# mobilinkd/m17-cxx-demod

Hardware: AMD Instinct MI355X
Metric: Msamples/s demodulated (48 kSPS 4-FSK in -> decoded frames) (higher is better)
Workload: dtype f32

## Files before the change

m17-cxx-demod_amd/csrc/m17_decode_device.hpp:

```cpp
#pragma once

#include "m17_common.hpp"

namespace m17 {

struct DecodeTables {
    uint16_t src[8][488];
    uint16_t lich_src[96];
    uint32_t golay_fix[2048];
};

__device__ __constant__ const int DEC_IN[4] = {488, 296, 420, 402};
__device__ __constant__ const int DEC_OUT[4] = {240, 144, 206, 197};

struct DecodeLds {
    uint32_t* llr;
    uint32_t* hist;
    uint32_t* outb;
    uint32_t* lsf;
    const uint16_t* src;
    const uint16_t* lich_src;
    int stride;
    int32_t* soft;
    unsigned long long* prof;
};

#define M17_LDS __attribute__((address_space(3)))
typedef uint32_t v4u __attribute__((ext_vector_type(4)));
template <typename T> __device__ __forceinline__ M17_LDS T* as_lds(T* p) { return (M17_LDS T*)p; }
template <typename T> __device__ __forceinline__ const M17_LDS T* as_lds(const T* p) { return (const M17_LDS T*)p; }
#define M17_GLOBAL __attribute__((address_space(1)))
template <typename T> __device__ __forceinline__ M17_GLOBAL T* as_global(T* p) { return (M17_GLOBAL T*)p; }
template <typename T> __device__ __forceinline__ T lds_get(const M17_LDS T* p)
{
    static_assert(sizeof(T) % 4 == 0, "word-sized structs only");
    T v;
    const M17_LDS uint32_t* s = reinterpret_cast<const M17_LDS uint32_t*>(p);
    uint32_t* d = reinterpret_cast<uint32_t*>(&v);
#pragma unroll
    for (int k = 0; k < (int)(sizeof(T) / 4); ++k) d[k] = s[k];
    return v;
}
template <typename T> __device__ __forceinline__ void lds_put(M17_LDS T* p, const T& v)
{
    static_assert(sizeof(T) % 4 == 0, "word-sized structs only");
    M17_LDS uint32_t* d = reinterpret_cast<M17_LDS uint32_t*>(p);
    const uint32_t* s = reinterpret_cast<const uint32_t*>(&v);
#pragma unroll
    for (int k = 0; k < (int)(sizeof(T) / 4); ++k) d[k] = s[k];
}

__device__ __forceinline__ int llr_at(const uint32_t* llr, int stride, int lane, int idx)
{
    const uint32_t w = llr[(idx >> 2) * stride + lane];
    return (int)(int8_t)(w >> (8 * (idx & 3)));
}
template <bool LQ = false>
__device__ __forceinline__ int llr_at_nib(const uint32_t* llr, int stride, int lane, int idx)
{
    const uint32_t w = LQ ? as_lds(llr)[(idx >> 3) * stride + lane] : llr[(idx >> 3) * stride + lane];
    return (int)(((w >> (4 * (idx & 7))) & 0xFu) ^ 8u) - 8;
}
template <bool NIB = false, bool LQ = false>
__device__ __forceinline__ int soft_at(const uint16_t* src, const uint32_t* llr, int stride, int lane, int kind, int i, int stale)
{
    const uint32_t e = LQ ? as_lds(src)[kind * 488 + i] : src[kind * 488 + i];
    if (LQ) {
        const int v = NIB ? llr_at_nib<LQ>(llr, stride, lane, (int)(e & 0x1FFu)) : llr_at(llr, stride, lane, (int)(e & 0x1FFu));
        const int w = (e & 0x200u) ? -v : v;
        return (e & 0x8000u) ? 0 : ((e & 0x4000u) ? stale : w);
    }
    if (e & 0x8000u) return 0;
    if (e & 0x4000u) return stale;
    const int v = NIB ? llr_at_nib<LQ>(llr, stride, lane, (int)(e & 0x1FFu)) : llr_at(llr, stride, lane, (int)(e & 0x1FFu));
    return (e & 0x200u) ? -v : v;
}
__device__ __forceinline__ uint32_t pack_llr_nibbles(uint32_t lo, uint32_t hi)
{
    auto four = [](uint32_t w) { return (w & 0xFu) | ((w >> 4) & 0xF0u) | ((w >> 8) & 0xF00u) | ((w >> 12) & 0xF000u); };
    return four(lo) | (four(hi) << 16);
}
__device__ __forceinline__ uint32_t unpack_llr_nibbles(uint32_t packed, int half)
{
    const uint32_t h = half ? packed >> 16 : packed & 0xFFFFu;
    uint32_t w = 0;
    for (int q = 0; q < 4; ++q) {
        const uint32_t n = (h >> (4 * q)) & 0xFu;
        w |= ((uint32_t)(uint8_t)(int8_t)((int)(n ^ 8u) - 8)) << (8 * q);
    }
    return w;
}
__device__ __forceinline__ uint32_t byte_at(const uint32_t* col, int stride, int lane, int b)
{
    return (col[(b >> 2) * stride + lane] >> (8 * (b & 3))) & 0xFFu;
}

__device__ __forceinline__ uint32_t crc16_col(const uint32_t* col, int stride, int lane, int n)
{
    uint32_t reg = 0xFFFFu;
    for (int i = 0; i != 16; ++i) {
        const uint32_t bit = reg & 1u;
        if (bit) reg ^= 0x5935u;
        reg >>= 1;
        if (bit) reg |= 0x8000u;
    }
    for (int k = 0; k < n; ++k) {
        const uint32_t byte = byte_at(col, stride, lane, k);
        for (int i = 0; i != 8; ++i) {
            const uint32_t msb = reg & 0x8000u;
            reg = ((reg << 1) & 0xFFFFu) | ((byte >> (7 - i)) & 1u);
            if (msb) reg ^= 0x5935u;
        }
    }
    for (int i = 0; i != 16; ++i) {
        const uint32_t msb = reg & 0x8000u;
        reg = (reg << 1) & 0xFFFFu;
        if (msb) reg ^= 0x5935u;
    }
    return reg;
}

__device__ __forceinline__ uint32_t golay_syndrome(uint32_t cw)
{
    cw &= 0xFFFFFFu;
    for (int i = 0; i != 12; ++i) {
        if (cw & 1u) cw ^= 0xC75u;
        cw >>= 1;
    }
    return cw;
}
__device__ __forceinline__ bool golay_decode(const DecodeTables* tb, uint32_t input, uint32_t& output)
{
    const uint32_t syn = golay_syndrome(input >> 1);
    const uint32_t correction = tb->golay_fix[syn & 0x7FFu] << 1;
    output = input ^ correction;
    return __popc(syn) < 3 || !(__popc(output) & 1);
}

template <bool NIB = false, bool LQ = false>
__device__ __forceinline__ uint32_t viterbi_decode(const DecodeTables* tb, const DecodeLds& L, int lane, int kind, int& stale_io)
{
    const int IN = DEC_IN[kind & 3], OUT = DEC_OUT[kind & 3];
    const int steps = IN >> 1;
    constexpr int32_t MAXM = 0x7FFFFFFF / 2;
    int32_t m[16];
#pragma unroll
    for (int s = 0; s < 16; ++s) m[s] = MAXM;
    m[0] = 0;
    uint32_t prev_bits = 0;
    int ns0 = soft_at<NIB, LQ>(L.src, L.llr, L.stride, lane, kind, 0, stale_io);
    int ns1 = soft_at<NIB, LQ>(L.src, L.llr, L.stride, lane, kind, 1, stale_io);
    for (int h = 0; h < steps; ++h) {
        const int s0 = ns0, s1 = ns1;
        if (2 * h == 400 && (kind & 3) != 3) stale_io = s1;
        if (h + 1 < steps) {
            ns0 = soft_at<NIB, LQ>(L.src, L.llr, L.stride, lane, kind, 2 * h + 2, stale_io);
            ns1 = soft_at<NIB, LQ>(L.src, L.llr, L.stride, lane, kind, 2 * h + 3, stale_io);
        }
        const int a = s0 ? abs(-7 - s0) : 0, b = s0 ? abs(7 - s0) : 0;
        const int d = s1 ? abs(-7 - s1) : 0, e = s1 ? abs(7 - s1) : 0;
        const uint32_t nn = 2u * (uint32_t)(a + d), np = 2u * (uint32_t)(a + e), pn = 2u * (uint32_t)(b + d), pp = 2u * (uint32_t)(b + e);
        const uint32_t c0[8] = {nn, np, np, nn, pn, pp, pp, pn};
        const uint32_t c1[8] = {pp, pn, pn, pp, np, nn, nn, np};
        uint32_t n[16];
        uint32_t bits = 0;
#pragma unroll
        for (int j = 0; j < 8; ++j) {
            const uint32_t lo = (uint32_t)m[j] << 1, hi = ((uint32_t)m[j + 8] << 1) + 1u;
            const uint32_t n0 = min(lo + c0[j], hi + c1[j]);
            const uint32_t n1 = min(lo + c1[j], hi + c0[j]);
            bits = __builtin_amdgcn_alignbit(n0, bits, 1);
            bits = __builtin_amdgcn_alignbit(n1, bits, 1);
            n[2 * j] = n0 >> 1;
            n[2 * j + 1] = n1 >> 1;
        }
#pragma unroll
        for (int s = 0; s < 16; ++s) m[s] = (int32_t)n[s];
        if (h & 1) {
            const uint32_t hw = prev_bits | (bits & 0xFFFF0000u);
            if (LQ) as_global(L.hist)[(h >> 1) * L.stride + lane] = hw;
            else L.hist[(h >> 1) * L.stride + lane] = hw;
        } else prev_bits = bits >> 16;
    }
    if (steps & 1) {
        if (LQ) as_global(L.hist)[(steps >> 1) * L.stride + lane] = prev_bits;
        else L.hist[(steps >> 1) * L.stride + lane] = prev_bits;
    }
    int best = 0;
    int32_t best_cost = m[0];
#pragma unroll
    for (int s = 1; s < 16; ++s)
        if (m[s] < best_cost) { best_cost = m[s]; best = s; }
    const uint32_t cost = (uint32_t)roundf((float)best_cost / 7.0f);
#pragma unroll
    for (int q = 0; q < 8; ++q) {
        if (LQ) as_lds(L.outb)[q * L.stride + lane] = 0;
        else L.outb[q * L.stride + lane] = 0;
    }
    uint32_t state = (uint32_t)best;
    uint32_t word = 0;
    int o = OUT;
    int index = steps;
    for (int hi = steps; hi > 0 && o > 0;) {
        --hi;
        const uint32_t hw = LQ ? as_global(L.hist)[(hi >> 1) * L.stride + lane] : L.hist[(hi >> 1) * L.stride + lane];
        const uint32_t hb = (hi & 1) ? (hw >> 16) : (hw & 0xFFFFu);
        const uint32_t v = (hb >> state) & 1u;
        if (index-- <= OUT) {
            --o;
            const int byte = o >> 3;
            word |= (state & 1u) << (8 * (byte & 3) + (7 - (o & 7)));
            if ((o & 31) == 0) {
                if (LQ) as_lds(L.outb)[(byte >> 2) * L.stride + lane] = word;
                else L.outb[(byte >> 2) * L.stride + lane] = word;
                word = 0;
            }
        }
        state = (state >> 1) + (v ? 8u : 0u);
    }
    return cost;
}

__device__ __forceinline__ uint32_t pk_add_bcast_lo(uint32_t p, uint32_t c)
{
    uint32_t r;
    asm("v_pk_add_u16 %0, %1, %2 op_sel:[0,0] op_sel_hi:[0,1]" : "=v"(r) : "v"(p), "v"(c));
    return r;
}
__device__ __forceinline__ uint32_t pk_add_bcast_hi(uint32_t p, uint32_t c)
{
    uint32_t r;
    asm("v_pk_add_u16 %0, %1, %2 op_sel:[1,0] op_sel_hi:[1,1]" : "=v"(r) : "v"(p), "v"(c));
    return r;
}
__device__ __forceinline__ uint32_t pk_min_u16(uint32_t a, uint32_t b)
{
    uint32_t r;
    asm("v_pk_min_u16 %0, %1, %2" : "=v"(r) : "v"(a), "v"(b));
    return r;
}
__device__ __forceinline__ uint32_t sad_u32(uint32_t a, uint32_t b, uint32_t c)
{
    uint32_t r;
    asm("v_sad_u32 %0, %1, %2, %3" : "=v"(r) : "v"(a), "v"(b), "v"(c));
    return r;
}
__device__ __forceinline__ uint32_t pk_sub_u16(uint32_t a, uint32_t b)
{
    uint32_t r;
    asm("v_pk_sub_u16 %0, %1, %2" : "=v"(r) : "v"(a), "v"(b));
    return r;
}
__device__ __forceinline__ uint32_t viterbi_decode_pk(const DecodeLds& L, int lane, int kind, int& stale_io)
{
    const int IN = DEC_IN[kind & 3], OUT = DEC_OUT[kind & 3];
    const int steps = IN >> 1;
    constexpr uint32_t SENT = 20000u;
    uint32_t P[8];
#pragma unroll
    for (int k = 0; k < 8; ++k) P[k] = SENT | (SENT << 16);
    P[0] = SENT << 16;
    const M17_LDS uint32_t* map2 = as_lds(reinterpret_cast<const uint32_t*>(L.src)) + kind * 244;
    const M17_LDS uint32_t* frame = as_lds(L.llr);
    auto ld_e = [&](int h) -> uint32_t { return h < steps ? map2[h] : 0x80008000u; };
    auto ld_w = [&](uint32_t e16) -> uint32_t { return frame[((e16 & 0x1FFu) >> 3) * L.stride + lane]; };
    auto mk_s = [&](uint32_t e16, uint32_t w) -> int {
        const int v = (int)(((w >> (4u * (e16 & 7u))) & 0xFu) ^ 8u) - 8;
        const int wv = (e16 & 0x200u) ? -v : v;
        return (e16 & 0x8000u) ? 0 : ((e16 & 0x4000u) ? stale_io : wv);
    };
    uint32_t e_cur = ld_e(0), e_nxt = ld_e(1);
    uint32_t wa = ld_w(e_cur & 0xFFFFu), wb = ld_w(e_cur >> 16);
    for (int h = 0; h < steps; ++h) {
        const int s0 = mk_s(e_cur & 0xFFFFu, wa), s1 = mk_s(e_cur >> 16, wb);
        if (2 * h == 400 && (kind & 3) != 3) stale_io = s1;
        const uint32_t e_nn2 = ld_e(h + 2);
        wa = ld_w(e_nxt & 0xFFFFu); wb = ld_w(e_nxt >> 16);
        e_cur = e_nxt; e_nxt = e_nn2;
        const uint32_t u0 = (uint32_t)(s0 + 8), u1 = (uint32_t)(s1 + 8);
        const uint32_t r0n = s0 ? 1u : u0, r0p = s0 ? 15u : u0, r1n = s1 ? 1u : u1, r1p = s1 ? 15u : u1;
        const uint32_t a = sad_u32(u0, r0n, 0u), b = sad_u32(u0, r0p, 0u);
        const uint32_t nn = sad_u32(u1, r1n, a), np = sad_u32(u1, r1p, a), pn = sad_u32(u1, r1n, b), pp = sad_u32(u1, r1p, b);
        const uint32_t e_nn = nn | (pp << 16), e_np = np | (pn << 16), e_pn = pn | (np << 16), e_pp = pp | (nn << 16);
        const uint32_t ce[8] = {e_nn, e_np, e_np, e_nn, e_pn, e_pp, e_pp, e_pn};
        const uint32_t co[8] = {e_pp, e_pn, e_pn, e_pp, e_np, e_nn, e_nn, e_np};
        uint32_t N[8];
        uint32_t acc = 0;
#pragma unroll
        for (int j = 0; j < 8; ++j) {
            const uint32_t x = (j & 1) ? pk_add_bcast_hi(P[j >> 1], ce[j]) : pk_add_bcast_lo(P[j >> 1], ce[j]);
            const uint32_t y = (j & 1) ? pk_add_bcast_hi(P[(j + 8) >> 1], co[j]) : pk_add_bcast_lo(P[(j + 8) >> 1], co[j]);
            N[j] = pk_min_u16(x, y);
            acc = (acc >> 1) | (pk_sub_u16(y, x) & 0x80008000u);
        }
#pragma unroll
        for (int k = 0; k < 8; ++k) P[k] = N[k];
        as_global(L.hist)[h * L.stride + lane] = acc;
    }
    auto metric = [&](int s) { return (int32_t)((s & 1) ? P[s >> 1] >> 16 : P[s >> 1] & 0xFFFFu); };
    int best = 0;
    int32_t best_cost = metric(0);
#pragma unroll
    for (int s = 1; s < 16; ++s) { const int32_t v = metric(s); if (v < best_cost) { best_cost = v; best = s; } }
    const uint32_t cost = (uint32_t)roundf((float)best_cost / 7.0f);
#pragma unroll
    for (int q = 0; q < 8; ++q) as_lds(L.outb)[q * L.stride + lane] = 0;
    uint32_t state = (uint32_t)best, word = 0;
    int o = OUT, index = steps;
    for (int top = steps; top > 0 && o > 0; top -= 16) {
        uint32_t hwv[16];
#pragma unroll
        for (int i = 0; i < 16; ++i) hwv[i] = as_global(L.hist)[max(top - 1 - i, 0) * L.stride + lane];
#pragma unroll
        for (int i = 0; i < 16; ++i) {
            if (top - 1 - i < 0 || o <= 0) break;
            const uint32_t v = (hwv[i] >> (8u + (state >> 1) + ((state & 1u) << 4))) & 1u;
            if (index-- <= OUT) {
                --o;
                const int byte = o >> 3;
                word |= (state & 1u) << (8 * (byte & 3) + (7 - (o & 7)));
                if ((o & 31) == 0) { as_lds(L.outb)[(byte >> 2) * L.stride + lane] = word; word = 0; }
            }
            state = (state >> 1) + (v ? 8u : 0u);
        }
    }
    return cost;
}

__device__ __forceinline__ void wave_lds_sync()
{
    __builtin_amdgcn_fence(__ATOMIC_RELEASE, "wavefront", "local");
    __builtin_amdgcn_wave_barrier();
    __builtin_amdgcn_fence(__ATOMIC_ACQUIRE, "wavefront", "local");
}
__device__ __forceinline__ int vit_pos_of_lane(int wl) { return (wl & 15) ^ ((wl & 4) ? 3 : 0); }
__device__ __forceinline__ int vit_lane_of_pos(int p) { return p ^ ((p & 4) ? 3 : 0); }
__device__ __forceinline__ int rotl4(int v, int r) { r &= 3; return ((v << r) | (v >> (4 - r))) & 15; }
__device__ __forceinline__ int rotr4(int v, int r) { return rotl4(v, 4 - (r & 3)); }

template <int R>
__device__ __forceinline__ int32_t vit_partner(int32_t m)
{
    if constexpr (R == 3) return __builtin_amdgcn_update_dpp(0, m, 0xB1, 0xF, 0xF, true);
    else if constexpr (R == 2) return __builtin_amdgcn_update_dpp(0, m, 0x4E, 0xF, 0xF, true);
    else if constexpr (R == 1) return __builtin_amdgcn_update_dpp(0, m, 0x141, 0xF, 0xF, true);
    else return __builtin_amdgcn_update_dpp(0, m, 0x128, 0xF, 0xF, true);
}

template <int R>
__device__ __forceinline__ uint32_t vit_step(uint32_t W, int wl, int32_t& m, uint32_t sh, unsigned long long upper)
{
    const int32_t c_own = (int32_t)__builtin_amdgcn_ubfe(W, sh, 8u);
    const int32_t c_oth = (int32_t)__builtin_amdgcn_ubfe(W, 24u - sh, 8u);
    const int32_t mp = vit_partner<R>(m);
    const int32_t own = m + c_own, oth = mp + c_oth;
    const int32_t low = ((upper >> wl) & 1ull) ? oth : own;
    m = min(own, oth);
    return (uint32_t)__ballot(m != low);
}

__device__ __forceinline__ uint32_t viterbi_decode_wave(const DecodeLds& L, int wl, int kind, int& stale_io)
{
    const int IN = DEC_IN[kind & 3], OUT = DEC_OUT[kind & 3];
    const int steps = IN >> 1;
    constexpr int32_t MAXM = 0x7FFFFFFF / 2;
    const unsigned long long tp0 = L.prof ? wall_clock64() : 0ull;
    M17_LDS uint32_t* cw = as_lds(reinterpret_cast<uint32_t*>(L.soft));
    M17_LDS uint32_t* hist = as_lds(L.hist);
    M17_LDS uint32_t* outb = as_lds(L.outb);
    {
        const uint16_t* src = L.src + kind * 488;
        const M17_LDS uint32_t* llr = as_lds(L.llr);
        auto soft = [&](uint32_t e) -> int {
            if (e & 0x8000u) return 0;
            if (e & 0x4000u) return stale_io;
            const uint32_t idx = e & 0x1FFu;
            const int v = (int)(int8_t)(llr[idx >> 2] >> (8 * (idx & 3)));
            return (e & 0x200u) ? -v : v;
        };
        int wlo = wl;
        asm volatile("" : "+v"(wlo));
        uint32_t e0 = wlo < steps ? src[2 * wlo] : 0x8000u, e1 = wlo < steps ? src[2 * wlo + 1] : 0x8000u;
        for (int h = wlo; h < steps; h += 64) {
            const int hn = h + 64;
            const uint32_t n0 = hn < steps ? src[2 * hn] : 0x8000u, n1 = hn < steps ? src[2 * hn + 1] : 0x8000u;
            const int s0 = soft(e0), s1 = soft(e1);
            const int a = s0 ? abs(-7 - s0) : 0, b = s0 ? abs(7 - s0) : 0;
            const int d = s1 ? abs(-7 - s1) : 0, e = s1 ? abs(7 - s1) : 0;
            cw[h] = (uint32_t)(a + d) | ((uint32_t)(a + e) << 8) | ((uint32_t)(b + d) << 16) | ((uint32_t)(b + e) << 24);
            if (h == 200) cw[480] = (uint32_t)s1;
            e0 = n0; e1 = n1;
        }
    }
    for (int h = steps + wl; h < ((steps + 3) & ~3); h += 64) cw[h] = 0;
    wave_lds_sync();
    if ((kind & 3) != 3 && IN > 401) stale_io = (int)cw[480];
    const int pos = vit_pos_of_lane(wl);
    uint32_t sh[4];
    unsigned long long upper[4];
#pragma unroll
    for (int r = 0; r < 4; ++r) {
        const int pb = 3 - r;
        upper[r] = __ballot((pos >> pb) & 1);
        const int j = rotl4(pos & ~(1 << pb), r);
        const bool c0neg = j < 4, c1neg = (((j ^ (j >> 1)) & 1) == 0);
        sh[r] = 8u * ((c0neg ? 0u : 2u) | (c1neg ? 0u : 1u));
    }
    int32_t m = (pos == 0) ? 0 : MAXM;
    const unsigned long long tp1 = L.prof ? wall_clock64() : 0ull;
    const int groups = (steps + 3) >> 2;
    v4u Wn = *reinterpret_cast<const M17_LDS v4u*>(cw);
    if (wl < 16)
    for (int g = 0; g < groups; ++g) {
        const v4u W = Wn;
        if (g + 1 < groups) Wn = *reinterpret_cast<const M17_LDS v4u*>(cw + 4 * (g + 1));
        const int h = 4 * g;
        const uint32_t b0 = vit_step<0>(W.x, wl, m, sh[0], upper[0]);
        int32_t m1 = m, m2, m3;
        const uint32_t b1 = vit_step<1>(W.y, wl, m1, sh[1], upper[1]);
        m2 = m1;
        const uint32_t b2 = vit_step<2>(W.z, wl, m2, sh[2], upper[2]);
        m3 = m2;
        const uint32_t b3 = vit_step<3>(W.w, wl, m3, sh[3], upper[3]);
        const int left = steps - h;
        m = left >= 4 ? m3 : (left == 3 ? m2 : (left == 2 ? m1 : m));
        hist[2 * g] = b0 | (b1 << 16);
        hist[2 * g + 1] = b2 | (b3 << 16);
    }
    const unsigned long long tp2 = L.prof ? wall_clock64() : 0ull;
    int best = 0;
    int32_t best_cost = __builtin_amdgcn_readlane(m, __builtin_amdgcn_readfirstlane(vit_lane_of_pos(rotr4(0, steps))));
#pragma unroll
    for (int s = 1; s < 16; ++s) {
        const int32_t v = __builtin_amdgcn_readlane(m, __builtin_amdgcn_readfirstlane(vit_lane_of_pos(rotr4(s, steps))));
        if (v < best_cost) { best_cost = v; best = s; }
    }
    const uint32_t cost = (uint32_t)roundf((float)best_cost / 7.0f);
    wave_lds_sync();
    for (int q = wl; q < 8; q += 64) outb[q] = 0;
    {
        auto to_pos_order = [](uint32_t x) -> uint32_t {
            const uint32_t odd = x & 0xF0F0F0F0u;
            return (x & 0x0F0F0F0Fu) | ((odd & 0x10101010u) << 3) | ((odd & 0x20202020u) << 1) | ((odd >> 1) & 0x20202020u) | ((odd >> 3) & 0x10101010u);
        };
        const int nreal = (steps + 1) >> 1;
        for (int q = wl; q < 130; q += 64) {
            const uint32_t neutral = (q & 1) ? 0xAAAACCCCu : 0xF0F0FF00u;
            uint32_t x = neutral;
            if (q < nreal) {
                x = to_pos_order(hist[q]);
                if (2 * q + 1 >= steps) x = (x & 0xFFFFu) | (neutral & 0xFFFF0000u);
            }
            cw[q] = x;
        }
    }
    wave_lds_sync();
    uint32_t I = (uint32_t)wl & 15u, w4 = 0, w4_hi = 0;
    {
        const M17_LDS uint32_t* hp = cw + 32 * (wl >> 4) + 2;
        auto rotr = [](uint32_t x, uint32_t n) -> uint32_t { return __builtin_amdgcn_alignbit(x, x, n); };
        auto take = [&](uint32_t prerot, uint32_t bit) {
            const uint32_t r = rotr(prerot, I);
            uint32_t out;
            asm("v_bfi_b32 %0, %1, %2, %3" : "=v"(out) : "v"(bit), "v"(r), "v"(I));
            I = out;
        };
#pragma unroll
        for (int g = 0; g < 16; ++g) {
            const uint32_t wa = hp[31 - 2 * g], wb = hp[30 - 2 * g];
// ... 234 lines not shown
```

m17-cxx-demod_amd/csrc/m17_parity_kernels.hpp:

```cpp
#pragma once

#include "m17_common.hpp"
#include "m17_decode_device.hpp"
#include "m17_state.hpp"

namespace m17 {

__global__ __launch_bounds__(64) void slice_kernel(const float* __restrict__ sym, uint32_t rows, uint32_t n, int8_t* __restrict__ llr,
                                                   float* __restrict__ evm, const float* __restrict__ edges)
{
    const uint32_t r = blockIdx.x * 64 + threadIdx.x;
    if (r >= rows) return;
    float S = 0.f;
    const float alpha = (float)(1.0 / 184);
    for (uint32_t k = 0; k < n; ++k) {
        const float sample = sym[(size_t)r * n + k];
        const uint32_t pair = slice_llr(sample, edges);
        llr[((size_t)r * n + k) * 2] = (int8_t)(pair & 0xFF);
        llr[((size_t)r * n + k) * 2 + 1] = (int8_t)(pair >> 8);
        float e;
        if (sample > 2.f) e = sample - 3.f;
        else if (sample > 0.f) e = sample - 1.f;
        else if (sample > -2.f) e = sample + 1.f;
        else e = sample + 3.f;
        S = S - S * alpha;
        S = S + (e * e) * alpha;
        evm[(size_t)r * n + k] = sqrtf(S);
    }
}

__global__ __launch_bounds__(64) void kalman_kernel(const float* __restrict__ z, const uint32_t* __restrict__ dt, uint32_t rows, uint32_t n, int wrap,
                                                    float z0, uint32_t order, float* __restrict__ out, const core::Kalman2Gain* __restrict__ gain)
{
    __shared__ Kal2 st[64];
    const uint32_t r = blockIdx.x * 64 + threadIdx.x;
    if (r >= rows) return;
    if (wrap == -1) {
        float x0 = z0, x1 = 0.f;
        for (uint32_t i = 0; i < n; ++i) {
            core::level_update(x0, x1, z[(size_t)r * n + i], gain[min(i, (uint32_t)core::LEVEL_SCHED_LAST)], order);
            float* o = out + ((size_t)r * n + i) * 6;
            o[0] = x0; o[1] = x1; o[2] = 0.f; o[3] = 0.f; o[4] = 0.f; o[5] = 0.f;
        }
        return;
    }
    M17_LDS Kal2* kp = as_lds(&st[threadIdx.x]);
    Kal2 k;
    kal_reset(k, z0);
    lds_put(kp, k);
    for (uint32_t i = 0; i < n; ++i) {
        kal_update(kp, z[(size_t)r * n + i], dt[(size_t)r * n + i], wrap, order);
        k = lds_get(kp);
        float* o = out + ((size_t)r * n + i) * 6;
        o[0] = k.x0; o[1] = k.x1; o[2] = k.p00; o[3] = k.p01; o[4] = k.p10; o[5] = k.p11;
    }
}

__global__ __launch_bounds__(64) void viterbi_kernel(const int8_t* __restrict__ soft, uint32_t n_frames, int kind,
                                                     uint8_t* __restrict__ bits, int32_t* __restrict__ cost,
                                                     const DecodeTables* ident)
{
    extern __shared__ __attribute__((aligned(16))) uint32_t lds[];
    DecodeLds L;
    L.llr = lds;
    L.hist = lds + 122 * 64;
    L.outb = L.hist + 122 * 64;
    L.lsf = L.outb + 8 * 64;
    L.stride = 64;
    L.prof = nullptr;
    L.src = &ident->src[0][0];
    L.lich_src = ident->lich_src;
    const int lane = threadIdx.x;
    const uint32_t f = blockIdx.x * 64 + lane;
    const int IN = DEC_IN[kind], OUT = DEC_OUT[kind];
    if (f < n_frames) {
        const int8_t* src = soft + (size_t)f * IN;
        for (int k = 0; k < (IN + 3) / 4; ++k) {
            uint32_t w = 0;
            for (int q = 0; q < 4; ++q)
                if (4 * k + q < IN) w |= (uint32_t)(uint8_t)src[4 * k + q] << (8 * q);
            L.llr[k * 64 + lane] = w;
        }
        int stale = llr_at(L.llr, 64, lane, kind == 3 ? 401 : 0);
        const uint32_t cst = viterbi_decode(ident, L, lane, kind + 4, stale);
        cost[f] = (int32_t)cst;
        for (int n = 0; n < OUT; ++n) bits[(size_t)f * OUT + n] = (uint8_t)((byte_at(L.outb, 64, lane, n >> 3) >> (7 - (n & 7))) & 1u);
    }
}

struct DecodeFramesParams {
    const int8_t* llr;
    const uint8_t* sync_type;
    uint8_t* state_io;
    uint8_t* lich_io;
    uint8_t* lsf_io;
    int8_t* dep401_io;
    int64_t* cost_io;
    FrameRec* recs;
    uint8_t* nrec;
    uint32_t n;
    const DecodeTables* tables;
    uint32_t* overflow;
};

__global__ __launch_bounds__(64) void decode_frames_kernel(DecodeFramesParams P)
{
    extern __shared__ __attribute__((aligned(16))) uint32_t lds[];
    DecodeLds L;
    L.llr = lds;
    L.hist = lds + 92 * 64;
    L.outb = L.hist + 122 * 64;
    L.lsf = L.outb + 8 * 64;
    L.stride = 64;
    L.prof = nullptr;
    L.src = &P.tables->src[0][0];
    L.lich_src = P.tables->lich_src;
    const int lane = threadIdx.x;
    const uint32_t f = blockIdx.x * 64 + lane;
    if (f >= P.n) return;
    const int8_t* src = P.llr + (size_t)f * 368;
    for (int k = 0; k < 92; ++k) {
        uint32_t w = 0;
        for (int q = 0; q < 4; ++q) w |= (uint32_t)(uint8_t)src[4 * k + q] << (8 * q);
        L.llr[k * 64 + lane] = w;
    }
    for (int k = 0; k < 8; ++k) {
        uint32_t w = 0;
        for (int q = 0; q < 4; ++q)
            if (4 * k + q < 30) w |= (uint32_t)P.lsf_io[(size_t)f * 30 + 4 * k + q] << (8 * q);
        L.lsf[k * 64 + lane] = w;
    }
    DecoderRegs D{P.state_io[f], P.lich_io[f], (int)P.dep401_io[f]};
    const int64_t cin = P.cost_io[f];
    uint32_t cost = cin < 0 ? 0xFFFFFFFFu : (uint32_t)cin;
    uint32_t n_run = 0, seq = 0;
    RecSink S{P.recs + (size_t)f * 2, 2, nullptr, nullptr, f, 0, P.sync_type[f], P.overflow};
    cost = decode_frame(P.tables, L, lane, P.sync_type[f], D, cost, S, n_run, seq);
    P.state_io[f] = (uint8_t)D.state;
    P.lich_io[f] = (uint8_t)D.lich_segments;
    P.dep401_io[f] = (int8_t)D.stale401;
    P.cost_io[f] = cost == 0xFFFFFFFFu ? (int64_t)-1 : (int64_t)cost;
    P.nrec[f] = (uint8_t)n_run;
    for (int k = 0; k < 30; ++k) P.lsf_io[(size_t)f * 30 + k] = (uint8_t)byte_at(L.lsf, 64, lane, k);
}

struct DeferParams {
    FrameRec* recs;
    uint32_t rec_cap;
    const uint32_t* rec_count;
    const uint32_t* defer;
    uint32_t* hist;
    const DecodeTables* tables;
    SeqState* state;
    Diag* diag_log;
    uint32_t diag_cap;
    const uint32_t* diag_count;
    uint32_t C;
    EvParams ev;
};
constexpr int DEFER_HIST_WORDS = 201;
constexpr int DEFER_CPB = 2;
constexpr int DEFER_WAVE_WORDS = (46 + 8) * 64 + 512 / 2;
constexpr int DEFER_LDS_BYTES = DEFER_CPB * DEFER_WAVE_WORDS * 4 + 4 * 488 * 2;
constexpr uint32_t defer_blocks(uint32_t C) { return (C + DEFER_CPB - 1) / DEFER_CPB; }
__global__ __launch_bounds__(64 * DEFER_CPB) void decode_deferred_kernel(DeferParams P)
{
    extern __shared__ __attribute__((aligned(16))) uint32_t lds[];
    if (blockIdx.x >= defer_blocks(P.C)) {
        if (threadIdx.x < 64) evm_fold_pass(P.ev, blockIdx.x - defer_blocks(P.C), reinterpret_cast<float*>(lds));
        return;
    }
    const int wave = __builtin_amdgcn_readfirstlane((int)(threadIdx.x >> 6));
    uint32_t* wb = lds + wave * DEFER_WAVE_WORDS;
    DecodeLds L;
    L.llr = wb;
    L.outb = wb + 46 * 64;
    uint16_t* list = reinterpret_cast<uint16_t*>(L.outb + 8 * 64);
    uint16_t* maps = reinterpret_cast<uint16_t*>(lds + DEFER_CPB * DEFER_WAVE_WORDS);
    L.lsf = nullptr;
    L.stride = 64;
    L.prof = nullptr;
    L.soft = nullptr;
    const int lane = threadIdx.x & 63;
    const uint32_t c = blockIdx.x * DEFER_CPB + wave;
    L.hist = P.hist + (size_t)c * DEFER_HIST_WORDS * 64;
    for (int k = threadIdx.x; k < 4 * 488; k += 64 * DEFER_CPB) maps[k] = P.tables->src[k / 488][k % 488];
    __syncthreads();
    L.src = maps;
    L.lich_src = P.tables->lich_src;
    if (c >= P.C) return;
    FrameRec* recs = P.recs + (size_t)c * P.rec_cap;
    const uint32_t n = min(P.rec_count[c], P.rec_cap);
    for (uint32_t s0 = 0; s0 < n; s0 += 512) {
        const uint32_t s1 = min(n, s0 + 512u);
        uint32_t nd = 0;
        wave_lds_sync();
        for (uint32_t base = s0; base < s1; base += 64) {
            const uint32_t slot = base + lane;
            bool d = false;
            if (slot < s1) {
                const uint32_t* w = reinterpret_cast<const uint32_t*>(recs + slot);
                d = cost_is_deferred(w[4]) && w[15] == DEFER_MARK;
            }
            const unsigned long long mask = __ballot(d);
            if (d) list[nd + __popcll(mask & ((1ull << lane) - 1ull))] = (uint16_t)(slot - s0);
            nd += (uint32_t)__popcll(mask);
        }
        wave_lds_sync();
        for (uint32_t k0 = lane; k0 < nd; k0 += 64) {
            const uint32_t slot = s0 + as_lds(list)[k0];
            uint32_t* w = reinterpret_cast<uint32_t*>(recs + slot);
            const uint32_t* src = P.defer + ((size_t)c * P.rec_cap + slot) * 46;
            for (int k = 0; k < 46; ++k) as_lds(L.llr)[k * 64 + lane] = src[k];
            const int kind = kind_of_frame_type(w[5] & 0xFFu);
            int stale = (int)w[14];
            const uint32_t cost = viterbi_decode_pk(L, lane, kind, stale);
            complete_record(w, cost, L.outb, 64, lane, len_of_kind(kind));
        }
    }
    __threadfence_block();
    wave_lds_sync();
    auto settle = [&](int32_t& v) {
        const uint32_t u = (uint32_t)v;
        if (cost_is_deferred(u)) v = recs[u & ~DEFER_TAG].cost;
    };
    if (P.diag_log) {
        const uint32_t nd = min(P.diag_count[c], P.diag_cap);
        Diag* log = P.diag_log + (size_t)c * P.diag_cap;
        for (uint32_t e = lane; e < nd; e += 64) settle(log[e].viterbi_cost);
    }
}

struct SettleParams {
    FrameRec* recs; uint32_t rec_cap; const uint32_t* defer; const DecodeTables* tables; SeqState* state; uint32_t C;
    EvParams ev;
};
constexpr int SETTLE_LDS_BYTES = (92 + 122 + 8 + 488) * 4 > EV_TILE_FLOATS * 4 ? (92 + 122 + 8 + 488) * 4 : EV_TILE_FLOATS * 4;
__global__ __launch_bounds__(64) void settle_tail_kernel(SettleParams P)
{
    extern __shared__ __attribute__((aligned(16))) uint32_t lds[];
    if (blockIdx.x >= P.C) {
        evm_fold_pass(P.ev, blockIdx.x - P.C, reinterpret_cast<float*>(lds));
        return;
    }
    const int wl = threadIdx.x;
    const uint32_t c = blockIdx.x;
    SeqState* st = P.state + c;
    const uint32_t th = (uint32_t)__builtin_amdgcn_readfirstlane((int)st->hot.viterbi_cost);
    const uint32_t td = (uint32_t)__builtin_amdgcn_readfirstlane(st->cold.diag.viterbi_cost);
    if (!cost_is_deferred(th) && !cost_is_deferred(td)) return;
    DecodeLds L;
    L.llr = lds; L.hist = lds + 92; L.outb = lds + 92 + 122; L.soft = reinterpret_cast<int32_t*>(lds + 92 + 122 + 8);
    L.lsf = nullptr; L.prof = nullptr; L.stride = 1;
    L.src = &P.tables->src[0][0]; L.lich_src = P.tables->lich_src;
    auto resolve = [&](uint32_t tag) -> uint32_t {
        const uint32_t slot = tag & ~DEFER_TAG;
        if (slot >= P.rec_cap) return 0u;
        uint32_t* w = reinterpret_cast<uint32_t*>(P.recs + (size_t)c * P.rec_cap + slot);
        const uint32_t have = (uint32_t)__builtin_amdgcn_readfirstlane((int)w[4]);
        if (!cost_is_deferred(have)) return have;
        const int kind = kind_of_frame_type(w[5] & 0xFFu);
        int stale = (int)w[14];
        const uint32_t* src = P.defer + ((size_t)c * P.rec_cap + slot) * 46;
        for (int k = wl; k < 92; k += 64) as_lds(L.llr)[k] = unpack_llr_nibbles(src[k >> 1], k & 1);
        wave_lds_sync();
        const uint32_t cost = viterbi_decode_wave(L, wl, kind, stale);
        wave_lds_sync();
        if (wl == 0) complete_record(w, cost, L.outb, 1, 0, len_of_kind(kind));
        wave_lds_sync();
        return cost;
    };
    uint32_t ch = th, cd = td;
    if (cost_is_deferred(th)) ch = resolve(th);
    if (cost_is_deferred(td)) cd = (td == th) ? ch : resolve(td);
    if (wl == 0) {
        st->hot.viterbi_cost = ch;
        st->cold.diag.viterbi_cost = (int32_t)cd;
    }
}

}
```

m17-cxx-demod_amd/csrc/m17hip.hip:

```cpp
#include "../../include/m17hip.h"

#include "m17_common.hpp"
#include "m17_decode_device.hpp"
#include "m17_frontend_kernels.hpp"
#include "m17_state.hpp"
#include "m17_wave_kernel.hpp"
#include "m17_gate_kernel.hpp"
#include "m17_mod_kernels.hpp"
#include "m17_parity_kernels.hpp"
#include "m17_gather.hpp"

#include <hip/hip_ext.h>

#include <algorithm>
#include <cmath>
#include <complex>
#include <cstdio>
#include <cstdlib>
#include <cstring>
#include <ctime>
#include <mutex>
#include <new>
#include <vector>

// ... 180 lines not shown
    uint32_t diag_cap = 0;
    uint32_t kalman_order = 3;
    int gather_fault = 0;
    uint32_t gather_timeout_ms = 120000;
    uint32_t channel_base = 0;
    uint32_t front_first = 0;
    int redo_form = 0;
    int dcd_form = -1;
    uint64_t seen_overlap = 0;
    hipEvent_t last_end = nullptr;
    uint32_t seg_len = 48000;
    uint32_t seg0_len = 0;
    int64_t seg_ramp = -1;
    DevBuf<DcdState> dcd_state;
    DevBuf<SeqState> seq_state;
    struct RecSet {
        DevBuf<FrameRec> recs;
        DevBuf<uint32_t> rec_count;
        DevBuf<uint32_t> defer_llr;
        uint32_t* ovf = nullptr;
        Event chain;
        Event done;
        uint32_t C = 0, rec_cap = 0, nseg = 0;
        bool valid = false;
        bool pending = false;
        bool bert = false, pkt = false;
    } sets[2];
    int cur = 0;
    uint32_t sel_back = 0;
    bool streams() const { return copy && slab[1].x; }
    hipStream_t pay() const { return streams() ? copy : stream; }
    Event ev_dst;
    Event ev_switch;
    Event ev_fetch;
    DevBuf<uint32_t> overflow;
    DevBuf<uint64_t> rec_offsets;
    DevBuf<FrameRec> compact;
    DevBuf<DecodeTables> tables;
    DevBuf<float> taps;
    DevBuf<float> taps_skew;
    int limit_form = 1;
    int fir_form = 1;
    int gate_aware = -1;
    DevBuf<GateTruth> truth;
    DevBuf<uint32_t> first_needed;
    uint32_t off_segs_prev = 0, chan_segs_prev = 0;
    uint32_t fir_grid = 0;
    uint32_t n_cu = 256;
    DevBuf<uint32_t> defer_hist;
    bool defer_decode = true;
    bool defer_evm = true;
    DevBuf<float> ev_ops2[2];
    int ev_par = 0;
    const float* fold_ops = nullptr;
    uint32_t fold_C = 0;
    const uint32_t* fold_end = nullptr;
    uint32_t ev_pitch = 0;
    uint32_t ev_pitch_override = 0;
    DevBuf<uint32_t> ev_cur;
    bool fold_pending = false;
    DevBuf<EvState> ev_state;
    uint32_t seq_lds_bytes = 0;
    DevBuf<float> llr_edges;
    DevBuf<core::Kalman2Gain> level_gain;
    DevBuf<char> scratch;
    DcdCoef coef{};
    uint64_t pos = 0;
    std::vector<uint32_t> marks;
    std::vector<uint8_t> marked;
    TurnTable reset_list;
    std::vector<uint8_t> pol_host;
    uint32_t pol_ones = 0;
    bool pol_dirty = false;
    TurnTable pol_table;
    uint32_t lastC = 0;
    bool have_run = false;
    bool uploaded = false;
    bool timing = false;
    bool profile = false;
    DevBuf<unsigned long long> dbg;
    uint32_t dbg_waves = 0;
    std::vector<TimedLaunch> pending;
    std::vector<Event> pool;
    double acc_ms[KT_N] = {0};
    uint64_t acc_n[KT_N] = {0};
};

struct m17hip_comm {
    ncclComm_t comm = nullptr;
    int device = 0;
    int rank = 0, nranks = 1;
    int last_rccl = 0;
    DevBuf<uint64_t> counts_dev;
    uint64_t* words_host = nullptr;
    uint32_t serial = 0;
    DevBuf<char> gathered;
    bool dead = false;
};

namespace {

#define HIPCHK(ctx, expr)                                   \
    do {                                                    \
        hipError_t e_ = (expr);                             \
        if (e_ != hipSuccess) {                             \
            (ctx)->last_hip = (int)e_;                      \
            return M17HIP_EHIP;                             \
        }                                                   \
    } while (0)

size_t round_up(size_t v, size_t m) { return (v + m - 1) / m * m; }

int alloc_code(m17hip_ctx* c, hipError_t e)
{
    if (e == hipSuccess) return M17HIP_OK;
    c->last_hip = (int)e;
    return e == hipErrorOutOfMemory ? M17HIP_ENOMEM : M17HIP_EHIP;
}

const uint8_t DC_SEQ[46] = {0xd6, 0xb5, 0xe2, 0x30, 0x82, 0xFF, 0x84, 0x62, 0xba, 0x4e, 0x96, 0x90, 0xd8, 0x98, 0xdd, 0x5d,
                            0x0c, 0xc8, 0x52, 0x43, 0x91, 0x1d, 0xf8, 0x6e, 0x68, 0x2F, 0x35, 0xda, 0x14, 0xea, 0xcd, 0x76,
                            0x19, 0x8d, 0xd5, 0x80, 0xd1, 0x33, 0x87, 0x13, 0x57, 0x18, 0x2d, 0x29, 0x78, 0xc3};

uint16_t frame_source(size_t deinterleaved_index)
{
    const size_t i = deinterleaved_index;
    const size_t src = (45 * i + 92 * i * i) % 368;
    const bool neg = (DC_SEQ[src >> 3] >> (7 - (src & 7))) & 1;
    return (uint16_t)(src | (neg ? 0x200u : 0u));
}

void build_tables(DecodeTables& t)
{
    std::memset(&t, 0, sizeof(t));
    std::vector<int> p1(61), p2(12, 1), p3(8, 1);
    for (size_t i = 0, j = 2; i != 61; ++i) { if (i == j) { p1[i] = 0; j += 4; } else p1[i] = 1; }
    p2[11] = 0;
    p3[7] = 0;
    struct Lay { int out, in, first; const std::vector<int>* p; };
    const Lay lay[4] = {{488, 368, 0, &p1}, {296, 272, 96, &p2}, {420, 368, 0, &p3}, {402, 368, 0, &p2}};
    for (int k = 0; k < 4; ++k) {
        size_t index = 0, pindex = 0;
        for (int i = 0; i < 488; ++i) t.src[k][i] = 0x8000;
        int i = 0;
        for (; i != lay[k].out && index < (size_t)lay[k].in; ++i) {
            if (!(*lay[k].p)[pindex++]) t.src[k][i] = 0x8000;
            else t.src[k][i] = frame_source(lay[k].first + index++);
            if (pindex == lay[k].p->size()) pindex = 0;
        }
        for (; i < lay[k].out; ++i) t.src[k][i] = 0x4000;
        for (int q = 0; q < 488; ++q) t.src[4 + k][q] = (uint16_t)q;
    }
    for (int i = 0; i < 96; ++i) t.lich_src[i] = frame_source(i);
    auto syndrome = [](uint32_t cw) { cw &= 0xFFFFFFu; for (int i = 0; i != 12; ++i) { if (cw & 1u) cw ^= 0xC75u; cw >>= 1; } return cw; };
    std::vector<int> seen(2048, 0);
    auto put = [&](uint32_t v) { const uint32_t s = syndrome(v) & 0x7FF; t.golay_fix[s] = v; seen[s]++; };
    put(0);
    for (int i = 0; i < 23; ++i) put(1u << i);
    for (int i = 0; i < 22; ++i) for (int j = i + 1; j < 23; ++j) put((1u << i) | (1u << j));
    for (int i = 0; i < 21; ++i) for (int j = i + 1; j < 22; ++j) for (int k = j + 1; k < 23; ++k) put((1u << i) | (1u << j) | (1u << k));
}

void build_llr_edges(float* e)
{
    const float inc = (float)(1.0 / (double)7.0f);
    float k = (float)(-3.0 + (double)inc);
    for (int n = 0; n < 43; ++n) { e[n] = k; k = k + inc; }
}

DcdCoef build_coef()
{
    const std::complex<float> j{0, 1};
    const float pi2 = (float)(M_PI * 2.0);
    auto coeff = [&](size_t f) { const float k = float(f) / float(48000); return std::exp(-j * pi2 * k); };
    const auto c0 = coeff(2400), c1 = coeff(3600);
    return DcdCoef{c0.real(), c0.imag(), c1.real(), c1.imag()};
}

Event get_event(m17hip_ctx* c)
{
    Event e;
    if (!c->pool.empty()) { e = std::move(c->pool.back()); c->pool.pop_back(); return e; }
    const hipError_t r = e.create(hipEventDefault);
    if (r != hipSuccess) c->last_hip = (int)r;
    return e;
}
void pool_events(m17hip_ctx* c, Event& a, Event& b)
{
    if (a) c->pool.push_back(std::move(a));
    if (b) c->pool.push_back(std::move(b));
}
struct Timed {
    m17hip_ctx* c; int which; hipStream_t st; Event a, b;
    Timed(m17hip_ctx* ctx, int w, hipStream_t stream) : c(ctx), which(w), st(stream)
    {
        if (!c->timing) return;
        a = get_event(c); b = get_event(c);
        if (!a || !b || hipEventRecord(a, st) != hipSuccess) pool_events(c, a, b);
    }
    Timed(m17hip_ctx* ctx, int w) : Timed(ctx, w, ctx->stream) {}
    ~Timed()
    {
        if (!a) return;
        if (hipEventRecord(b, st) == hipSuccess) c->pending.push_back({std::move(a), std::move(b), which});
        else pool_events(c, a, b);
    }
};
struct TimedK {
    m17hip_ctx* c; int which; Event a, b;
    TimedK(m17hip_ctx* ctx, int w) : c(ctx), which(w)
    {
        if (!c->timing) return;
        a = get_event(c); b = get_event(c);
        if (!a || !b) pool_events(c, a, b);
    }
    ~TimedK() { if (a) c->pending.push_back({std::move(a), std::move(b), which}); }
    template <typename... P, typename... A>
    void launch(void (*kernel)(P...), dim3 grid, dim3 block, uint32_t lds, hipStream_t st, const A&... args)
    {
        if (a) hipExtLaunchKernelGGL(kernel, grid, block, lds, st, a, b, 0, static_cast<P>(args)...);
        else hipLaunchKernelGGL(kernel, grid, block, lds, st, static_cast<P>(args)...);
    }
};
struct DeviceGuard {
    int prev = -1; bool ok = true;
    explicit DeviceGuard(m17hip_ctx* c)
    {
        if (hipGetDevice(&prev) != hipSuccess) prev = -1;
        if (prev != c->device) { const hipError_t e = hipSetDevice(c->device); if (e != hipSuccess) { c->last_hip = (int)e; ok = false; prev = -1; } }
        else prev = -1;
        (void)hipGetLastError();
    }
    ~DeviceGuard() { if (prev >= 0) hipSetDevice(prev); }
};
#define GUARD(ctx) DeviceGuard guard_(ctx); if (!guard_.ok) return M17HIP_EHIP

struct RunRegistry { std::mutex mu; std::vector<m17hip_ctx*> ctxs; uint64_t overlaps = 0; };
RunRegistry& g_runs_ref() { static RunRegistry* r = new RunRegistry; return *r; }
#define g_runs (g_runs_ref())
bool runs_overlap(m17hip_ctx* c)
{
    std::lock_guard<std::mutex> lk(g_runs.mu);
    bool other = false;
    for (m17hip_ctx* o : g_runs.ctxs)
        if (o != c && o->device == c->device && o->last_end && hipEventQuery(o->last_end) == hipErrorNotReady) other = true;
    (void)hipGetLastError();
    if (other) ++g_runs.overlaps;
    const bool overlapped = other || g_runs.overlaps != c->seen_overlap;
    c->seen_overlap = g_runs.overlaps;
    return overlapped;
}
void drain_timing(m17hip_ctx* c)
{
    for (auto& t : c->pending) {
        hipEventSynchronize(t.b);
        float ms = 0.f;
        if (hipEventElapsedTime(&ms, t.a, t.b) == hipSuccess) { c->acc_ms[t.which] += ms; c->acc_n[t.which]++; }
        pool_events(c, t.a, t.b);
    }
    c->pending.clear();
}

__global__ void ev_move_kernel(SeqState* st, EvState* es, uint32_t C, int to_deferred)
{
    const uint32_t c = blockIdx.x * blockDim.x + threadIdx.x;
    if (c >= C) return;
    if (to_deferred) { es[c].S = st[c].hot.evm_S; es[c].pos = 0; } else st[c].hot.evm_S = es[c].S;
}

__device__ __forceinline__ void fresh_demod_state(SeqState* st, EvState* es, uint32_t c, uint64_t pos)
{
    es[c] = EvState{1.0f, 0.f, 0u, 0u};
    uint32_t* w = reinterpret_cast<uint32_t*>(st + c);
    for (size_t k = 0; k < sizeof(SeqState) / 4; ++k) w[k] = 0;
    Hot& s = st[c].hot;
    Cold& k = st[c].cold;
    s.run_pos = 148;
    kal_reset(k.ck, 0.f);
    k.dev_reset = 1;
    s.evm_S = 1.0f;
    s.initializing = 1920;
    s.st = ST_UNLOCKED;
    k.seg_start_tick = (uint32_t)(pos / TICK);
    k.origin_lo = (uint32_t)pos; k.origin_hi = (uint32_t)(pos >> 32);
}
__device__ __forceinline__ void fresh_dcd_state(DcdState* ds, uint32_t c)
{
    uint32_t* d = reinterpret_cast<uint32_t*>(ds + c);
    for (size_t k = 0; k < sizeof(DcdState) / 4; ++k) d[k] = 0;
}

__global__ void seq_reset_kernel(SeqState* st, DcdState* ds, EvState* es, uint32_t C)
{
    const uint32_t c = blockIdx.x * blockDim.x + threadIdx.x;
    if (c >= C) return;
    fresh_demod_state(st, es, c, 0);
    fresh_dcd_state(ds, c);
}

__global__ void front_reset_list_kernel(const uint32_t* list, uint32_t n, int16_t* x, size_t xpitch, DcdState* ds)
{
    if (blockIdx.x >= n) return;
    const uint32_t c = list[blockIdx.x];
    if (x) for (int k = threadIdx.x; k < XPRE; k += blockDim.x) x[(size_t)c * xpitch + k] = 0;
    if (ds && threadIdx.x == 0) fresh_dcd_state(ds, c);
}
// ... 2281 lines not shown
```

Baseline: 102,800.

## Precompute packed Viterbi input map and compute branch metrics with packed i16 ops

Replaces the per-step 16-bit source map decode (mask tests, shift, sign flip, sad-based metrics) with a host-built 32-bit map whose entries hold shift, row offset and sign multiplier. Branch metrics are then formed with bfe plus packed i16 mad/abs, and the four pair costs come from op_sel variants of one packed add. The survivor history word is now assembled by byte permutes instead of a serial shift-or chain, and the traceback bit index is changed to match. The stale-bit handling moves to an LDS row, and the deferred kernel stages only the stream and BERT maps, which shrinks LDS so more waves can fit per CU. In exchange the decode depends on a new table layout and a reordered history bit format.

```diff
diff --git a/m17-cxx-demod_amd/csrc/m17_decode_device.hpp b/m17-cxx-demod_amd/csrc/m17_decode_device.hpp
--- a/m17-cxx-demod_amd/csrc/m17_decode_device.hpp
+++ b/m17-cxx-demod_amd/csrc/m17_decode_device.hpp
@@ -8,7 +8,18 @@
     uint16_t src[8][488];
     uint16_t lich_src[96];
     uint32_t golay_fix[2048];
+    uint32_t pk_map[706];
 };
+constexpr int PK_MAP_STREAM = 0, PK_MAP_BERT = 296 + 4, PK_MAP_WORDS = PK_MAP_BERT + 402 + 4;
+constexpr uint32_t PK_ROW_STALE = 46;
+static_assert(PK_MAP_WORDS == 706 && PK_MAP_BERT % 2 == 0, "DecodeTables::pk_map");
+constexpr uint32_t pk_map_entry(uint16_t e)
+{
+    if (e & 0x8000u) return 0u;
+    if (e & 0x4000u) return (PK_ROW_STALE << 8) | (1u << 16);
+    const uint32_t idx = e & 0x1FFu;
+    return (4u * (idx & 7u)) | ((idx >> 3) << 8) | ((e & 0x200u) ? 0xFFFF0000u : 0x00010000u);
+}
 
 __device__ __constant__ const int DEC_IN[4] = {488, 296, 420, 402};
 __device__ __constant__ const int DEC_OUT[4] = {240, 144, 206, 197};
@@ -239,19 +250,47 @@
     asm("v_pk_min_u16 %0, %1, %2" : "=v"(r) : "v"(a), "v"(b));
     return r;
 }
-__device__ __forceinline__ uint32_t sad_u32(uint32_t a, uint32_t b, uint32_t c)
-{
-    uint32_t r;
-    asm("v_sad_u32 %0, %1, %2, %3" : "=v"(r) : "v"(a), "v"(b), "v"(c));
-    return r;
-}
 __device__ __forceinline__ uint32_t pk_sub_u16(uint32_t a, uint32_t b)
 {
     uint32_t r;
     asm("v_pk_sub_u16 %0, %1, %2" : "=v"(r) : "v"(a), "v"(b));
     return r;
 }
-__device__ __forceinline__ uint32_t viterbi_decode_pk(const DecodeLds& L, int lane, int kind, int& stale_io)
+__device__ __forceinline__ uint32_t pk_add_u16(uint32_t a, uint32_t b)
+{
+    uint32_t r;
+    asm("v_pk_add_u16 %0, %1, %2" : "=v"(r) : "v"(a), "v"(b));
+    return r;
+}
+__device__ __forceinline__ uint32_t pk_add_u16_xb(uint32_t a, uint32_t b)
+{
+    uint32_t r;
+    asm("v_pk_add_u16 %0, %1, %2 op_sel:[0,1] op_sel_hi:[1,0]" : "=v"(r) : "v"(a), "v"(b));
+    return r;
+}
+__device__ __forceinline__ uint32_t pk_add_u16_xa(uint32_t a, uint32_t b)
+{
+    uint32_t r;
+    asm("v_pk_add_u16 %0, %1, %2 op_sel:[1,0] op_sel_hi:[0,1]" : "=v"(r) : "v"(a), "v"(b));
+    return r;
+}
+__device__ __forceinline__ uint32_t pk_add_u16_xab(uint32_t a, uint32_t b)
+{
+    uint32_t r;
+    asm("v_pk_add_u16 %0, %1, %2 op_sel:[1,1] op_sel_hi:[0,0]" : "=v"(r) : "v"(a), "v"(b));
+    return r;
+}
+__device__ __forceinline__ uint32_t pk_bit_metrics(uint32_t w, uint32_t e)
+{
+    constexpr uint32_t K = 0xFFF90007u;
+    uint32_t v, x, nx, ax;
+    asm("v_bfe_i32 %0, %1, %2, 4" : "=v"(v) : "v"(w), "v"(e));
+    asm("v_pk_mad_i16 %0, %1, %2, %3 op_sel:[0,1,0] op_sel_hi:[0,1,1]" : "=v"(x) : "v"(v), "v"(e), "s"(K));
+    asm("v_pk_sub_i16 %0, 0, %1" : "=v"(nx) : "v"(x));
+    asm("v_pk_max_i16 %0, %1, %2" : "=v"(ax) : "v"(x), "v"(nx));
+    return x != K ? ax : 0u;
+}
+__device__ __forceinline__ uint32_t viterbi_decode_pk(const DecodeLds& L, const uint32_t* pk_map, int lane, int kind, int stale)
 {
     const int IN = DEC_IN[kind & 3], OUT = DEC_OUT[kind & 3];
     const int steps = IN >> 1;
@@ -260,42 +299,39 @@
 #pragma unroll
     for (int k = 0; k < 8; ++k) P[k] = SENT | (SENT << 16);
     P[0] = SENT << 16;
-    const M17_LDS uint32_t* map2 = as_lds(reinterpret_cast<const uint32_t*>(L.src)) + kind * 244;
-    const M17_LDS uint32_t* frame = as_lds(L.llr);
-    auto ld_e = [&](int h) -> uint32_t { return h < steps ? map2[h] : 0x80008000u; };
-    auto ld_w = [&](uint32_t e16) -> uint32_t { return frame[((e16 & 0x1FFu) >> 3) * L.stride + lane]; };
-    auto mk_s = [&](uint32_t e16, uint32_t w) -> int {
-        const int v = (int)(((w >> (4u * (e16 & 7u))) & 0xFu) ^ 8u) - 8;
-        const int wv = (e16 & 0x200u) ? -v : v;
-        return (e16 & 0x8000u) ? 0 : ((e16 & 0x4000u) ? stale_io : wv);
-    };
-    uint32_t e_cur = ld_e(0), e_nxt = ld_e(1);
-    uint32_t wa = ld_w(e_cur & 0xFFFFu), wb = ld_w(e_cur >> 16);
+    typedef uint32_t v2u __attribute__((ext_vector_type(2)));
+    const M17_LDS v2u* map2 = reinterpret_cast<const M17_LDS v2u*>(as_lds(pk_map) + ((kind & 3) == 3 ? PK_MAP_BERT : PK_MAP_STREAM));
+    const M17_LDS char* col = reinterpret_cast<const M17_LDS char*>(as_lds(L.llr) + lane);
+    as_lds(L.outb)[lane] = (uint32_t)stale;
+    auto ld_w = [&](uint32_t e) -> uint32_t { return *reinterpret_cast<const M17_LDS uint32_t*>(col + (e & 0x3F00u)); };
+    v2u e_cur = map2[0], e_nxt = map2[1];
+    uint32_t wa = ld_w(e_cur.x), wb = ld_w(e_cur.y);
+    M17_GLOBAL uint32_t* hist = as_global(L.hist) + lane;
     for (int h = 0; h < steps; ++h) {
-        const int s0 = mk_s(e_cur & 0xFFFFu, wa), s1 = mk_s(e_cur >> 16, wb);
-        if (2 * h == 400 && (kind & 3) != 3) stale_io = s1;
-        const uint32_t e_nn2 = ld_e(h + 2);
-        wa = ld_w(e_nxt & 0xFFFFu); wb = ld_w(e_nxt >> 16);
+        const uint32_t a0 = pk_bit_metrics(wa, e_cur.x), a1 = pk_bit_metrics(wb, e_cur.y);
+        const v2u e_nn2 = map2[h + 2];
+        wa = ld_w(e_nxt.x); wb = ld_w(e_nxt.y);
         e_cur = e_nxt; e_nxt = e_nn2;
-        const uint32_t u0 = (uint32_t)(s0 + 8), u1 = (uint32_t)(s1 + 8);
-        const uint32_t r0n = s0 ? 1u : u0, r0p = s0 ? 15u : u0, r1n = s1 ? 1u : u1, r1p = s1 ? 15u : u1;
-        const uint32_t a = sad_u32(u0, r0n, 0u), b = sad_u32(u0, r0p, 0u);
-        const uint32_t nn = sad_u32(u1, r1n, a), np = sad_u32(u1, r1p, a), pn = sad_u32(u1, r1n, b), pp = sad_u32(u1, r1p, b);
-        const uint32_t e_nn = nn | (pp << 16), e_np = np | (pn << 16), e_pn = pn | (np << 16), e_pp = pp | (nn << 16);
+        const uint32_t e_nn = pk_add_u16(a0, a1), e_np = pk_add_u16_xb(a0, a1), e_pn = pk_add_u16_xa(a0, a1), e_pp = pk_add_u16_xab(a0, a1);
         const uint32_t ce[8] = {e_nn, e_np, e_np, e_nn, e_pn, e_pp, e_pp, e_pn};
         const uint32_t co[8] = {e_pp, e_pn, e_pn, e_pp, e_np, e_nn, e_nn, e_np};
-        uint32_t N[8];
-        uint32_t acc = 0;
+        uint32_t N[8], D[8];
 #pragma unroll
         for (int j = 0; j < 8; ++j) {
             const uint32_t x = (j & 1) ? pk_add_bcast_hi(P[j >> 1], ce[j]) : pk_add_bcast_lo(P[j >> 1], ce[j]);
             const uint32_t y = (j & 1) ? pk_add_bcast_hi(P[(j + 8) >> 1], co[j]) : pk_add_bcast_lo(P[(j + 8) >> 1], co[j]);
             N[j] = pk_min_u16(x, y);
-            acc = (acc >> 1) | (pk_sub_u16(y, x) & 0x80008000u);
+            D[j] = pk_sub_u16(y, x);
         }
 #pragma unroll
         for (int k = 0; k < 8; ++k) P[k] = N[k];
-        as_global(L.hist)[h * L.stride + lane] = acc;
+        uint32_t g[4];
+#pragma unroll
+        for (int t = 0; t < 4; ++t) g[t] = __builtin_amdgcn_perm(D[2 * t + 1], D[2 * t], 0x07050301u);
+        uint32_t acc = (g[2] >> 2 & 0x20202020u) | (g[3] >> 3 & ~0x20202020u);
+        acc = (g[1] >> 1 & 0x40404040u) | (acc & ~0x40404040u);
+        acc = (g[0] & 0x80808080u) | (acc & ~0x80808080u);
+        hist[h * L.stride] = acc;
     }
     auto metric = [&](int s) { return (int32_t)((s & 1) ? P[s >> 1] >> 16 : P[s >> 1] & 0xFFFFu); };
     int best = 0;
@@ -314,7 +350,7 @@
 #pragma unroll
         for (int i = 0; i < 16; ++i) {
             if (top - 1 - i < 0 || o <= 0) break;
-            const uint32_t v = (hwv[i] >> (8u + (state >> 1) + ((state & 1u) << 4))) & 1u;
+            const uint32_t v = (hwv[i] >> (((state & 3u) << 3) + 7u - (state >> 2))) & 1u;
             if (index-- <= OUT) {
                 --o;
                 const int byte = o >> 3;
diff --git a/m17-cxx-demod_amd/csrc/m17_parity_kernels.hpp b/m17-cxx-demod_amd/csrc/m17_parity_kernels.hpp
--- a/m17-cxx-demod_amd/csrc/m17_parity_kernels.hpp
+++ b/m17-cxx-demod_amd/csrc/m17_parity_kernels.hpp
@@ -161,7 +161,8 @@
 constexpr int DEFER_HIST_WORDS = 201;
 constexpr int DEFER_CPB = 2;
 constexpr int DEFER_WAVE_WORDS = (46 + 8) * 64 + 512 / 2;
-constexpr int DEFER_LDS_BYTES = DEFER_CPB * DEFER_WAVE_WORDS * 4 + 4 * 488 * 2;
+constexpr int DEFER_LDS_BYTES = (DEFER_CPB * DEFER_WAVE_WORDS + PK_MAP_WORDS) * 4;
+static_assert(5 * DEFER_LDS_BYTES <= 160 * 1024, "ten waves per CU");
 constexpr uint32_t defer_blocks(uint32_t C) { return (C + DEFER_CPB - 1) / DEFER_CPB; }
 __global__ __launch_bounds__(64 * DEFER_CPB) void decode_deferred_kernel(DeferParams P)
 {
@@ -176,7 +177,7 @@
     L.llr = wb;
     L.outb = wb + 46 * 64;
     uint16_t* list = reinterpret_cast<uint16_t*>(L.outb + 8 * 64);
-    uint16_t* maps = reinterpret_cast<uint16_t*>(lds + DEFER_CPB * DEFER_WAVE_WORDS);
+    uint32_t* maps = lds + DEFER_CPB * DEFER_WAVE_WORDS;
     L.lsf = nullptr;
     L.stride = 64;
     L.prof = nullptr;
@@ -184,9 +185,9 @@
     const int lane = threadIdx.x & 63;
     const uint32_t c = blockIdx.x * DEFER_CPB + wave;
     L.hist = P.hist + (size_t)c * DEFER_HIST_WORDS * 64;
-    for (int k = threadIdx.x; k < 4 * 488; k += 64 * DEFER_CPB) maps[k] = P.tables->src[k / 488][k % 488];
+    for (int k = threadIdx.x; k < PK_MAP_WORDS; k += 64 * DEFER_CPB) maps[k] = P.tables->pk_map[k];
     __syncthreads();
-    L.src = maps;
+    L.src = &P.tables->src[0][0];
     L.lich_src = P.tables->lich_src;
     if (c >= P.C) return;
     FrameRec* recs = P.recs + (size_t)c * P.rec_cap;
@@ -213,8 +214,7 @@
             const uint32_t* src = P.defer + ((size_t)c * P.rec_cap + slot) * 46;
             for (int k = 0; k < 46; ++k) as_lds(L.llr)[k * 64 + lane] = src[k];
             const int kind = kind_of_frame_type(w[5] & 0xFFu);
-            int stale = (int)w[14];
-            const uint32_t cost = viterbi_decode_pk(L, lane, kind, stale);
+            const uint32_t cost = viterbi_decode_pk(L, maps, lane, kind, (int)w[14]);
             complete_record(w, cost, L.outb, 64, lane, len_of_kind(kind));
         }
     }
diff --git a/m17-cxx-demod_amd/csrc/m17hip.hip b/m17-cxx-demod_amd/csrc/m17hip.hip
--- a/m17-cxx-demod_amd/csrc/m17hip.hip
+++ b/m17-cxx-demod_amd/csrc/m17hip.hip
@@ -356,6 +356,8 @@
         for (int q = 0; q < 488; ++q) t.src[4 + k][q] = (uint16_t)q;
     }
     for (int i = 0; i < 96; ++i) t.lich_src[i] = frame_source(i);
+    for (int i = 0; i < 296 + 4; ++i) t.pk_map[PK_MAP_STREAM + i] = pk_map_entry(t.src[1][i]);
+    for (int i = 0; i < 402 + 4; ++i) t.pk_map[PK_MAP_BERT + i] = pk_map_entry(t.src[3][i]);
     auto syndrome = [](uint32_t cw) { cw &= 0xFFFFFFu; for (int i = 0; i != 12; ++i) { if (cw & 1u) cw ^= 0xC75u; cw >>= 1; } return cw; };
     std::vector<int> seen(2048, 0);
     auto put = [&](uint32_t v) { const uint32_t s = syndrome(v) & 0x7FF; t.golay_fix[s] = v; seen[s]++; };
```

Result: no change. 103,700 (median of 6 runs) (+0.9%).
